# etemesi254/zune-jpeg

Measured on AMD Instinct MI355X. Metric: megapixels/sec decoded (IDCT->RGB), 4K 4:2:0 baseline, higher is better.
Workload: dtype i32

## Files before the change

### zune-jpeg_amd/csrc/zj_device.h

```cpp
#pragma once

#include <stdint.h>

#if defined(ZJ_EMU)
#define ZJ_DEV inline
#define ZJ_HD inline
#else
#include <hip/hip_runtime.h>
#define ZJ_DEV __device__ __forceinline__
#define ZJ_HD __host__ __device__ __forceinline__
#endif

namespace zj {

typedef uint16_t u16x2 __attribute__((vector_size(4)));
typedef int16_t s16x2 __attribute__((vector_size(4)));

#if defined(ZJ_EMU)
#define ZJ_GLOBAL_PTR(T, v) (reinterpret_cast<T*>(v))
#else
#define ZJ_GLOBAL_PTR(T, v) ((T*)(__attribute__((address_space(1))) T*)(v))
#endif

struct alignas(16) U4 { uint32_t x, y, z, w; };
struct alignas(8) U2 { uint32_t x, y; };
typedef uint32_t V4 __attribute__((vector_size(16)));
#if defined(ZJ_ABLATION)
#define ZJ_ABL(debug, bit) ((debug) & (bit))
#define ZJ_PDBG(p) ((p).debug)
#else
#define ZJ_ABL(debug, bit) 0
#define ZJ_PDBG(p) 0
#endif
#ifndef ZJ_NT
#define ZJ_NT 4
#endif
#ifndef ZJ_SEAM_WB
#define ZJ_SEAM_WB 0
#endif
#ifndef ZJ_ROUND_ROT
#define ZJ_ROUND_ROT 1
#endif

#ifndef ZJ_CBYTE
#define ZJ_CBYTE 1
#endif
#ifndef ZJ_INTERIOR
#define ZJ_INTERIOR 1
#endif

ZJ_DEV uint32_t as_u32(u16x2 v) { uint32_t r; __builtin_memcpy(&r, &v, 4); return r; }
ZJ_DEV uint32_t as_u32(s16x2 v) { uint32_t r; __builtin_memcpy(&r, &v, 4); return r; }
ZJ_DEV u16x2 as_u16x2(uint32_t v) { u16x2 r; __builtin_memcpy(&r, &v, 4); return r; }
ZJ_DEV s16x2 as_s16x2(uint32_t v) { s16x2 r; __builtin_memcpy(&r, &v, 4); return r; }

#if !defined(ZJ_EMU)
extern "C" __device__ __attribute__((const)) int zj_llvm_mul_i24(int, int) __asm("llvm.amdgcn.mul.i24");
#endif
ZJ_DEV int32_t mul24(int32_t a, int32_t b)
{
#if defined(ZJ_EMU)
    int32_t a24 = (int32_t)((uint32_t)a << 8) >> 8, b24 = (int32_t)((uint32_t)b << 8) >> 8;
    return (int32_t)((uint32_t)a24 * (uint32_t)b24);
#else
    return zj_llvm_mul_i24(a, b);
#endif
}
ZJ_DEV int32_t wadd(int32_t a, int32_t b) { return (int32_t)((uint32_t)a + (uint32_t)b); }
ZJ_DEV int32_t wsub(int32_t a, int32_t b) { return (int32_t)((uint32_t)a - (uint32_t)b); }
ZJ_DEV int32_t mad24(int32_t a, int32_t b, int32_t c) { return wadd(mul24(a, b), c); }
ZJ_DEV int32_t wshl(int32_t a, int s) { return (int32_t)((uint32_t)a << s); }

ZJ_DEV int32_t dot2(uint32_t a, uint32_t k, int32_t c)
{
#if defined(ZJ_EMU)
    const int32_t al = (int16_t)(a & 0xffff), ah = (int16_t)(a >> 16), bl = (int16_t)(k & 0xffff), bh = (int16_t)(k >> 16);
    return (int32_t)((uint32_t)(al * bl) + (uint32_t)(ah * bh) + (uint32_t)c);
#else
    int32_t r;
    asm("v_dot2_i32_i16 %0, %1, %2, %3" : "=v"(r) : "v"(a), "s"(k), "v"(c));
    return r;
#endif
}
ZJ_DEV int32_t dot2z(uint32_t a, uint32_t k)
{
#if defined(ZJ_EMU)
    return dot2(a, k, 0);
#else
    int32_t r;
    asm("v_dot2_i32_i16 %0, %1, %2, 0" : "=v"(r) : "v"(a), "s"(k));
    return r;
#endif
}
constexpr uint32_t pk16(int lo, int hi) { return ((uint32_t)lo & 0xffffu) | (((uint32_t)hi & 0xffffu) << 16); }

ZJ_DEV uint32_t sad_u16(uint32_t a, uint32_t b, uint32_t c)
{
#if defined(ZJ_EMU)
    const int32_t al = (int32_t)(a & 0xffff), ah = (int32_t)(a >> 16), bl = (int32_t)(b & 0xffff), bh = (int32_t)(b >> 16);
    return (uint32_t)((al > bl ? al - bl : bl - al) + (ah > bh ? ah - bh : bh - ah)) + c;
#else
// ... 240 lines not shown
#pragma unroll
        for (int g = 0; g < G; g++)
#pragma unroll
            for (int k = 0; k < 8; k += 2) {
                const uint32_t hi = perm((uint32_t)o[g][k + 1], (uint32_t)o[g][k], 0x07060302u);
                const s16x2 z = {0, 0}, m = {255, 255};
                ow[(r0 + g) * 4 + (k >> 1)] = as_u32(pk_min(pk_max(sar(as_u16x2(hi), 1), z), m));
            }
        ZJ_SCHED_BARRIER();
    }
}

struct PackedHalf { int32_t x0, x1, x2, x3, u0, u1, u2, u3; };
ZJ_DEV PackedHalf idct_1d_dot(const uint32_t p04, const uint32_t p26, const uint32_t p13, const uint32_t p57, const int32_t bias)
{
    PackedHalf h;
    const int32_t t0 = dot2(p04, pk16(4096, 4096), bias);
    const int32_t t1 = dot2(p04, pk16(4096, -4096), bias);
    h.x0 = dot2(p26, pk16(5352, 2217), t0);
    h.x3 = dot2(p26, pk16(-5352, -2217), t0);
    h.x1 = dot2(p26, pk16(2217, -5350), t1);
    h.x2 = dot2(p26, pk16(-2217, 5350), t1);
    h.u3 = dot2(p57, pk16(3219, 1131), dot2z(p13, pk16(5683, 4816)));
    h.u2 = dot2(p57, pk16(-5681, -3218), dot2z(p13, pk16(4816, -1129)));
    h.u1 = dot2(p57, pk16(1132, 4816), dot2z(p13, pk16(3219, -5681)));
    h.u0 = dot2(p57, pk16(4816, -5680), dot2z(p13, pk16(1131, -3218)));
    return h;
}
ZJ_DEV void idct_1d_dot_add(const PackedHalf& h, int32_t o[8])
{
    o[0] = wadd(h.x0, h.u3); o[7] = wsub(h.x0, h.u3);
    o[1] = wadd(h.x1, h.u2); o[6] = wsub(h.x1, h.u2);
    o[2] = wadd(h.x2, h.u1); o[5] = wsub(h.x2, h.u1);
    o[3] = wadd(h.x3, h.u0); o[4] = wsub(h.x3, h.u0);
}

ZJ_DEV int classify_block(const uint32_t* w, const uint32_t* g)
{
    uint32_t any = w[0] & 0xffff0000u;
#pragma unroll
    for (int i = 1; i < 32; i++) any |= w[i];
    if (any == 0) return 0;
    int32_t bad = 0;
#pragma unroll
    for (int jj = 0; jj < 4; jj++) {
        uint32_t st = 0, sb = 0;
#pragma unroll
        for (int k = 0; k < 4; k++) st = sad_u16(w[4 * k + jj], 0x80008000u, st);
#pragma unroll
        for (int k = 4; k < 8; k++) sb = sad_u16(w[4 * k + jj], 0x80008000u, sb);
        const int32_t d = mad24((int32_t)g[4 + jj], (int32_t)sb, mad24((int32_t)g[jj], (int32_t)st, -(int32_t)g[8 + jj]));
        bad |= d;
    }
    return bad < 0 ? 2 : 1;
}

ZJ_DEV void idct_block_packed(const U4 raw[8], const uint32_t* qp, uint32_t out[16])
{
    const uint32_t* w = reinterpret_cast<const uint32_t*>(raw);
    uint32_t D[32];
#pragma unroll
    for (int i = 0; i < 32; i++) D[i] = as_u32(as_u16x2(w[i]) * as_u16x2(qp[i]));
    uint32_t T[8][4];
#pragma unroll
    for (int g = 0; g < 4; g++) {
        const int ca = g == 0 ? 0 : (g == 1 ? 2 : (g == 2 ? 1 : 5)), cb = g == 0 ? 4 : (g == 1 ? 6 : (g == 2 ? 3 : 7));
        PackedHalf h[2];
#pragma unroll
        for (int e = 0; e < 2; e++) {
            const int col = e ? cb : ca, jj = col >> 1;
            const uint32_t sel = (col & 1) ? 0x07060302u : 0x05040100u;
            const uint32_t p04 = perm(D[4 * 4 + jj], D[0 * 4 + jj], sel), p26 = perm(D[6 * 4 + jj], D[2 * 4 + jj], sel);
            const uint32_t p13 = perm(D[3 * 4 + jj], D[1 * 4 + jj], sel), p57 = perm(D[7 * 4 + jj], D[5 * 4 + jj], sel);
            h[e] = idct_1d_dot(p04, p26, p13, p57, 512);
        }
        ZJ_SCHED_BARRIER();
        int32_t oa[8], ob[8];
        idct_1d_dot_add(h[0], oa);
        idct_1d_dot_add(h[1], ob);
#pragma unroll
        for (int i = 0; i < 8; i++) T[i][g] = pack_sar<10>(oa[i], ob[i]);
        ZJ_SCHED_BARRIER();
    }
    constexpr int32_t bias2 = 512 + 65536 + (128 << 17);
#pragma unroll
    for (int r0 = 0; r0 < 8; r0 += 2) {
        PackedHalf h[2];
#pragma unroll
        for (int e = 0; e < 2; e++) h[e] = idct_1d_dot(T[r0 + e][0], T[r0 + e][1], T[r0 + e][2], T[r0 + e][3], bias2);
        ZJ_SCHED_BARRIER();
#pragma unroll
        for (int e = 0; e < 2; e++) {
            int32_t o[8];
            idct_1d_dot_add(h[e], o);
            out[2 * (r0 + e)] = sat_pk_u8_2(pack_sar<17>(o[0], o[1]), pack_sar<17>(o[2], o[3]));
            out[2 * (r0 + e) + 1] = sat_pk_u8_2(pack_sar<17>(o[4], o[5]), pack_sar<17>(o[6], o[7]));
        }
        ZJ_SCHED_BARRIER();
    }
}

ZJ_DEV uint32_t dc_only_value(uint32_t w0, int32_t q0, const int clamp = 0)
{
    const int16_t dc = (int16_t)(uint16_t)((uint32_t)lo16s(w0) * (uint32_t)(int32_t)(int16_t)q0);
    int32_t v = ((int32_t)dc >> 3) + 128;
    if (clamp) v = v < 0 ? 0 : (v > 255 ? 255 : v);
// ... 56 lines not shown
#define ZJ_TWC_GRAY 128
#endif
#ifndef ZJ_NT_MIN_GRAY
#define ZJ_NT_MIN_GRAY 256
#endif
template <> struct TileWidth<1, 1, false> { static constexpr int TWC = ZJ_TWC_GRAY; };

enum { OUT_RGB = 0, OUT_GRAY = 1, OUT_YCBCR = 2, OUT_RGBA = 3, OUT_RGB_CHW = 4 };
enum { GEN_WIDE = 0, GEN_PACKED = 1 };

template <int HS, int VS, int OUT>
struct Cfg {
    static constexpr bool CHROMA = OUT != OUT_GRAY;
    static constexpr int YBR = (HS == 2 && VS == 2) ? 4 : ((HS == 2 || VS == 2) ? 2 : 1);
    static constexpr int CBR = (HS == 2) ? 2 : 1;
    static constexpr int SH = YBR * 8;
    static constexpr int CROWS = CBR * 8;
    static constexpr int TWC = TileWidth<HS, VS, CHROMA>::TWC;
    static constexpr int HALO = (HS == 2) ? 1 : 0;
    static constexpr int TWYB = TWC * HS;
    static constexpr int TWY = TWYB * 8;
    static constexpr int NYB = YBR * TWYB;
    static constexpr int CCOLS = TWC + 2 * HALO;
    static constexpr int NCB = CBR * CCOLS;
    static constexpr int CPITCH = TWC * 8;
    static constexpr int COFF = 0;
    static constexpr int YSZ = SH * TWY;
    static constexpr int CSZ = CROWS * CPITCH;
    static constexpr int NGRP = TWY / 16;
    static constexpr int NITEMS = SH * NGRP;
    static constexpr int NBLK = NYB + (CHROMA ? 2 * NCB : 0);
    static constexpr int NT_BLK = (NBLK + 63) / 64 * 64;
    static constexpr int NT_MIN = (HS == 1 && VS == 1) ? (CHROMA ? ZJ_NT_MIN_444 : ZJ_NT_MIN_GRAY) : ((HS == 2 && VS == 1 && CHROMA) ? ZJ_NT_MIN_H : ((HS == 2 && VS == 2 && CHROMA) ? ZJ_NT_MIN_HV : ((HS == 1 && VS == 2 && CHROMA) ? ZJ_NT_MIN_V : 0)));
    static constexpr int NT = NT_BLK > NT_MIN ? NT_BLK : NT_MIN;
    static constexpr int NW = NT / 64;
    static constexpr int ROUND_ROT = (ZJ_ROUND_ROT && NITEMS % NT != 0 && NITEMS % NT <= 64 && NW > 1) ? 1 : 0;

    static constexpr int LUT_N = SH + 2;
    static constexpr int LUT_BYTES = ((2 * LUT_N * 2 + 15) / 16) * 16;
    static constexpr int HRAW = (CHROMA && HALO) ? 2 * 2 * CROWS : 0;
    static constexpr int HFIL = (CHROMA && HALO) ? 2 * 2 * SH : 0;
    static constexpr bool TSCAP = OUT == OUT_RGB || OUT == OUT_YCBCR || OUT == OUT_RGBA;
    static constexpr int PPI = OUT == OUT_RGBA ? 4 : 3;
    static constexpr int INPL = 64 / PPI * PPI;
    static constexpr int XSTAGE = ((64 * PPI - INPL) * 16 + 31) / 32 * 32;
    static constexpr bool HALO_PURE = CHROMA && HALO && (NYB + 2 * CBR * TWC) % 64 == 0 && 2 * CBR * 2 * 8 == 64;
    static constexpr int HALO_T0 = NYB + 2 * CBR * TWC;
#if defined(ZJ_EMU) && !defined(ZJ_EMU_REDO_ANY)
    static constexpr bool CBYTE_OUT = OUT == OUT_RGB || OUT == OUT_RGBA || OUT == OUT_RGB_CHW;
#else
    static constexpr bool CBYTE_OUT = true;
#endif
    static constexpr bool CBYTE = ZJ_CBYTE != 0 && CHROMA && HS == 2 && HALO_PURE && NGRP == 16 && NYB % 64 == 0 && CBYTE_OUT;
    static constexpr bool INTERIOR = ZJ_INTERIOR != 0 && CBYTE && TSCAP && NITEMS % NT == 0 && ROUND_ROT == 0;
    template <int GEN> struct L {
        static constexpr int YPX = GEN == GEN_PACKED ? 1 : 2;
        static constexpr bool CB = GEN == GEN_PACKED && CBYTE;
        static constexpr int CPX = CB ? 1 : 2;
        static constexpr int CPB = CPITCH * CPX;
        static constexpr int CPLANE = CROWS * CPB;
        static constexpr int CBYTES = CHROMA ? 2 * CPLANE + (HRAW + HFIL) * 2 : 0;
        static_assert(CBYTES % 16 == 0, "tables stay 16-byte aligned");
        static constexpr int C_OFF = GEN == GEN_PACKED ? (NITEMS + 63) / 64 * 64 * 16 : YSZ * 2;
        static constexpr int HRAW_OFF = C_OFF + 2 * CPLANE;
        static constexpr int HFIL_OFF = HRAW_OFF + HRAW * 2;
        static constexpr int TAB_OFF = C_OFF + CBYTES;
        static constexpr int LUT_OFF = TAB_OFF + TAB_BYTES;
        static constexpr int FLAG_OFF = LUT_OFF + LUT_BYTES;
        static constexpr int X_OFF = FLAG_OFF + 16;
        static constexpr int X_STAGE = TSCAP ? NW * XSTAGE : 0;
        static constexpr int X_HALO = HALO_PURE ? 8 * 80 * 4 : 0;
        static constexpr int BYTES = GEN == GEN_PACKED ? X_OFF + (X_STAGE > X_HALO ? X_STAGE : X_HALO) : FLAG_OFF;
        static_assert(C_OFF % 16 == 0 && TAB_OFF % 16 == 0, "16-byte alignment of the planes");
    };
    static constexpr int LDS_WIDE = L<GEN_WIDE>::BYTES;
    static constexpr int LDS_PACKED = L<GEN_PACKED>::BYTES > LDS_WIDE ? L<GEN_PACKED>::BYTES : LDS_WIDE;
    static constexpr int PIECES_PER_ROW = PPI * NGRP;
    static constexpr int PPR_MAGIC = (1 << 20) / PIECES_PER_ROW + 1;
    static constexpr bool ppr_magic_ok()
    {
        for (int q = 0; q < PPI * ((NITEMS + NT - 1) / NT * NT) + 64 * PPI; q++)
            if ((int)(((unsigned)q * (unsigned)PPR_MAGIC) >> 20) != q / PIECES_PER_ROW) return false;
        return true;
    }
    static_assert(ppr_magic_ok(), "PPR_MAGIC");
    static_assert(NT <= 512 && NBLK <= NT, "one lane per block, at most 8 waves");
};

constexpr int SCATTER_MAX = 32;

struct Params {
    const int16_t* y;
    const int16_t* cb;
    const int16_t* cr;
    uint8_t* out;
    long long y_frame_stride;
    long long c_frame_stride;
    long long out_frame_stride;
    int width, height;
    int mcu_x;
    int n_strips;
    int tiles_per_row;
    int regular_px;
    int nframes;
    int zero_fill;
    int total_tiles;
    uint32_t tpr_magic, tpr_shift;
// ... 296 lines not shown
template <class C>
ZJ_DEV void halo_pass2(const HaloLane& H, char* lds, const int clamp_dc)
{
    const int32_t* sc = lds_halo_scratch<C>(lds, H.hb);
    const int i = H.j;
    const U4 f0 = *reinterpret_cast<const U4*>(sc + 64), f1 = *reinterpret_cast<const U4*>(sc + 68);
    const uint32_t any = f0.x | f0.y | f0.z | f0.w | f1.x | f1.y | f1.z | f1.w;
    int32_t v;
    if (any == 0) {
        const uint16_t* q = reinterpret_cast<const uint16_t*>(lds_tab<C, GEN_PACKED>(lds) + TAB_DW * H.comp);
        v = (int32_t)(int16_t)(dc_only_value((uint32_t)sc[72], (int32_t)q[0], clamp_dc) & 0xffffu);
        if (C::template L<GEN_PACKED>::CB && (uint32_t)v > 255u) *lds_flag<C>(lds) = 1;
    } else {
        const U4 a = *reinterpret_cast<const U4*>(sc + 8 * i), b = *reinterpret_cast<const U4*>(sc + 8 * i + 4);
        const int32_t t0 = (int32_t)a.x, t1 = (int32_t)a.y, t2 = (int32_t)a.z, t3 = (int32_t)a.w;
        const int32_t t4 = (int32_t)b.x, t5 = (int32_t)b.y, t6 = (int32_t)b.z, t7 = (int32_t)b.w;
        constexpr int32_t bias2 = 512 + 65536 + (128 << 17);
        int32_t x0 = mad24(t2, 2217 + 3135, wadd(wshl(wadd(t0, t4), 12), bias2));
        x0 = mad24(t6, 2217, x0);
        int32_t u3 = mul24(t1, 6149 + 4816 - 3685 - 1597);
        u3 = mad24(t7, 4816 - 3685, u3);
        u3 = mad24(t5, 4816 - 1597, u3);
        u3 = mad24(t3, 4816, u3);
        v = (H.last_col ? wsub(x0, u3) : wadd(x0, u3)) >> 17;
        v = v < 0 ? 0 : (v > 255 ? 255 : v);
    }
    *reinterpret_cast<int16_t*>(H.dst + i * H.pitch) = (int16_t)v;
}

template <class C, int HS, int VS, int GEN>
ZJ_DEV int halo_value(char* lds, const int comp, const int side, const int m, const bool wrap)
{
    const int16_t* raw = lds_halo_raw<C, GEN>(lds, comp, side, 0);
    if (VS == 2) {
        const int16_t* lut = lds_lut<C, GEN>(lds);
        const int i = m + 1 + (wrap ? (side == 0 ? -1 : 1) : 0);
        const int ra = lut[i] / C::template L<GEN>::CPB, rb = lut[C::LUT_N + i] / C::template L<GEN>::CPB;
        return tri1(raw[ra], raw[rb]);
    }
    const int r = side == 0 ? (wrap && m > 0 ? m - 1 : m) : (wrap && m < C::SH - 1 ? m + 1 : m);
    return raw[r];
}
template <class C, int HS, int VS>
ZJ_DEV void halo_filter(const Params& p, const TileId t, const int hl, char* lds)
{
    const int cbw = p.mcu_x, cb0 = t.tile * C::TWC;
    const bool left_wrap = cb0 == 0, right_wrap = cb0 + C::TWC >= cbw;
    for (int q = hl; q < C::HFIL; q += 64) {
        const int comp = 1 + q / (2 * C::SH), side = (q / C::SH) & 1, m = q % C::SH;
        *lds_halo_fil<C, GEN_PACKED>(lds, comp, side, m) = (int16_t)halo_value<C, HS, VS, GEN_PACKED>(lds, comp, side, m, side == 0 ? left_wrap : right_wrap);
    }
}

template <class C, int GEN, bool NEED_Y16>
ZJ_DEV void finish_block(const BlockLoc& L, const U4 raw[8], char* lds, const int debug = 0, const int clamp_dc = 0)
{
    if (!L.valid) return;
    const uint32_t* w = reinterpret_cast<const uint32_t*>(raw);
    const uint32_t* tab = lds_tab<C, GEN>(lds) + TAB_DW * L.comp;
    if (GEN == GEN_WIDE) {
        uint32_t any = w[0] & 0xffff0000u;
#pragma unroll
        for (int i = 1; i < 32; i++) any |= w[i];
        if (any != 0 && !ZJ_ABL(debug, 1)) {
            U4 px[8];
            idct_block(raw, reinterpret_cast<const uint16_t*>(tab), px);
            store_block(L, px);
        } else {
            store_splat(L, dc_only_value(w[0], (int32_t)(tab[0] & 0xffffu), clamp_dc));
        }
        return;
    }
    using LLp = typename C::template L<GEN_PACKED>;
    constexpr bool CB = LLp::CB;
    constexpr bool CONST_PITCH = C::HALO_PURE && (CB || C::TWY * LLp::YPX == LLp::CPB);
    BlockLoc Lc = L;
    if (CONST_PITCH) { Lc.pitch = LLp::CPB; Lc.halo = 0; }
    const int ypitch = CONST_PITCH ? C::TWY * LLp::YPX : L.pitch;
    int cls = classify_block(w, tab + 32);
    if (ZJ_ABL(debug, 1)) cls = 0;
    if (cls == 0) {
        const uint32_t v = dc_only_value(w[0], (int32_t)(tab[0] & 0xffffu), clamp_dc);
        if (L.comp != 0 && !CB) { store_splat(Lc, v); return; }
        if ((L.comp != 0 || NEED_Y16) && (v & 0xffffu) > 255u) *lds_flag<C>(lds) = 1;
        const uint32_t b = (v & 0xffu) * 0x01010101u;
        const U2 row = {b, b};
        if (L.comp != 0) {
#pragma unroll
            for (int r = 0; r < 8; r++) *reinterpret_cast<U2*>(Lc.dst + r * Lc.pitch) = row;
            return;
        }
#pragma unroll
        for (int r = 0; r < 8; r++) *reinterpret_cast<U2*>(Lc.dst + r * ypitch) = row;
        return;
    }
    auto emit = [&](const uint32_t* b) {
        if (L.comp == 0) {
#pragma unroll
            for (int r = 0; r < 8; r++) { const U2 row = {b[2 * r], b[2 * r + 1]}; *reinterpret_cast<U2*>(Lc.dst + r * ypitch) = row; }
        } else if (CB) {
#pragma unroll
            for (int r = 0; r < 8; r++) { const U2 row = {b[2 * r], b[2 * r + 1]}; *reinterpret_cast<U2*>(Lc.dst + r * Lc.pitch) = row; }
        } else {
            U4 px[8];
            bytes_to_rows(b, px);
            store_block(Lc, px);
        }
    };
    if (cls == 1) {
        uint32_t b[16];
        idct_block_packed(raw, tab, b);
        emit(b);
        return;
    }
    {
        ZJ_NO_IF_CONVERT();
        uint32_t b[16];
        U4 px[8];
        idct_block(raw, reinterpret_cast<const uint16_t*>(tab), px);
        rows_to_bytes(px, b);
        emit(b);
    }
}

ZJ_DEV void store16(uint8_t* p, const U4& v, const bool staged = false)
{
#if !defined(ZJ_EMU)
    if ((ZJ_NT & 1) || ((ZJ_NT & 4) && staged)) { const V4 t = {v.x, v.y, v.z, v.w}; __builtin_nontemporal_store(t, reinterpret_cast<V4*>(p)); return; }
#endif
#if defined(ZJ_EMU)
    __builtin_memcpy(p, &v, 16);
#else
// ... 113 lines not shown
    return (q < C::INPL ? ybase : xbase) + 16 * q;
}

template <class C, int VS>
ZJ_DEV void nb_pair(const uint32_t vm[4], const char* cp, const int oa, const int ob, const int lc, const int g, uint32_t& prev, uint32_t& next,
                    const uint32_t pl = 0, const uint32_t nr = 0)
{
#if !defined(ZJ_EMU)
    if (C::NGRP == 16) {
        prev = (uint32_t)__builtin_amdgcn_update_dpp((int)pl, (int)vm[3], 0x111, 0xf, 0xf, false);
        next = (uint32_t)__builtin_amdgcn_update_dpp((int)nr, (int)vm[0], 0x101, 0xf, 0xf, false);
        return;
    }
#endif
    prev = next = 0;
    if (g > 0) {
        prev = *reinterpret_cast<const uint32_t*>(cp + oa + lc - 4);
        if (VS == 2) prev = tri(prev, *reinterpret_cast<const uint32_t*>(cp + ob + lc - 4));
    }
    if (g < C::NGRP - 1) {
        next = *reinterpret_cast<const uint32_t*>(cp + oa + lc + 16);
        if (VS == 2) next = tri(next, *reinterpret_cast<const uint32_t*>(cp + ob + lc + 16));
    }
}

template <class C, int VS>
ZJ_DEV void nb_bytes(const uint32_t a0, const uint32_t a1, const char* cp, const int oa, const int ob, const int lc, const int g,
                     uint32_t& prev, uint32_t& next, const uint32_t pl, const uint32_t nr)
{
#if !defined(ZJ_EMU)
    if (C::NGRP == 16) {
        prev = (uint32_t)__builtin_amdgcn_update_dpp((int)pl, (int)a1, 0x111, 0xf, 0xf, false);
        next = (uint32_t)__builtin_amdgcn_update_dpp((int)nr, (int)a0, 0x101, 0xf, 0xf, false);
        return;
    }
#endif
    prev = next = 0;
    if (g > 0) {
        prev = *reinterpret_cast<const uint32_t*>(cp + oa + lc - 4);
        if (VS == 2) prev = tri_b(prev, *reinterpret_cast<const uint32_t*>(cp + ob + lc - 4));
    }
    if (g < C::NGRP - 1) {
        next = *reinterpret_cast<const uint32_t*>(cp + oa + lc + 8);
        if (VS == 2) next = tri_b(next, *reinterpret_cast<const uint32_t*>(cp + ob + lc + 8));
    }
}

template <class C>
ZJ_DEV bool interior_tile(const Params& p, const TileId t)
{
    const int cb0 = t.tile * C::TWC;
    return cb0 != 0 && cb0 + C::TWC < p.mcu_x && p.height - t.strip * C::SH >= C::SH && p.edge_rep == 0;
}

template <class C, bool INTERIOR = false>
ZJ_DEV void stage_item(const ItemOut& io, const int tid , char* lds, const int round, const int hw_wave = -1)
{
    if (!INTERIOR && io.kind == 0) return;
    const int lwave = tid >> 6, lane = tid & 63;
    const int item0 = 64 * lwave + round * C::NT;
    const int wave = hw_wave < 0 ? lwave : hw_wave;
    if (!INTERIOR && C::PPI == 3 && io.kind == 3) {
        const U4 z = {0, 0, 0, 0};
        *reinterpret_cast<U4*>(piece_addr<C>(lds, item0, wave, 3 * lane - 1)) = io.s0;
        *reinterpret_cast<U4*>(piece_addr<C>(lds, item0, wave, 3 * lane)) = io.s1;
        *reinterpret_cast<U4*>(piece_addr<C>(lds, item0, wave, 3 * lane + 1)) = io.s2;
        *reinterpret_cast<U4*>(piece_addr<C>(lds, item0, wave, 3 * lane + 2)) = z;
        return;
    }
    U4* const dst = reinterpret_cast<U4*>(piece_addr<C>(lds, item0, wave, C::PPI * lane));
    dst[0] = io.s0;
    dst[1] = io.s1;
    if (C::PPI == 4) { dst[2] = io.s2; dst[3] = io.s3; }
    else if (INTERIOR || io.kind == 1) dst[2] = io.s2;
}

template <class C, int HS, int VS, int OUT, int GEN, bool FAST = true, bool TS = false, bool RAG = false, bool INTERIOR = false>
ZJ_DEV void phase_color(const Params& p, const TileId t, const int tid, char* lds, const int round = 0, ItemOut* io = nullptr)
{
    using LL = typename C::template L<GEN>;
    static_assert(!INTERIOR || (TS && FAST && !RAG && GEN == GEN_PACKED && LL::CB && C::INTERIOR), "the interior form exists for the staged byte-chroma rounds");
    const int P = p.mcu_x * 8 * HS;
    const int W = p.width;
    const int cbw = p.mcu_x;
    const int cb0 = t.tile * C::TWC;
    const int nvalid = INTERIOR ? C::TWC : ((cbw - cb0) < C::TWC ? (cbw - cb0) : C::TWC);
    const bool left_wrap = !INTERIOR && cb0 == 0, right_wrap = !INTERIOR && cb0 + C::TWC >= cbw;
    const bool edge_tile = HS == 2 && (left_wrap || right_wrap);
    const int x0 = t.tile * C::TWY;
    const long long row_bytes = p.out_pitch;
    uint8_t* const frame_out = t.out;
    const int elements = P / 16 - 1;
    if (TS) io->kind = 0;

    for (int item = TS ? tid + round * C::NT : tid; item < C::NITEMS; item += TS ? C::NITEMS : C::NT) {
        const int m = item / C::NGRP, g = item % C::NGRP;
        const int px0 = x0 + 16 * g;
        const int row = t.strip * C::SH + m;
        if (!INTERIOR && (px0 >= P || row >= p.height)) continue;
        const bool irregular = RAG && px0 >= p.regular_px;
        uint8_t* const orow = frame_out + (long long)row * row_bytes;
        uint32_t yp[8];
        if (GEN == GEN_PACKED) {
            const U4 yv = *reinterpret_cast<const U4*>(lds + 16 * item);
            if (OUT == OUT_GRAY) {
                if (FAST && !irregular) store16(orow + px0, yv, true);
                else { const uint32_t ow4[4] = {yv.x, yv.y, yv.z, yv.w}; store_clip(orow, px0, ow4, 4, W, 0, 0); }
                continue;
            }
            const uint32_t yb[4] = {yv.x, yv.y, yv.z, yv.w};
#pragma unroll
            for (int k = 0; k < 4; k++) {
                if (HS == 2) { yp[k] = perm(0, yb[k], 0x0c020c00u); yp[4 + k] = perm(0, yb[k], 0x0c030c01u); }
                else { yp[2 * k] = perm(0, yb[k], 0x0c010c00u); yp[2 * k + 1] = perm(0, yb[k], 0x0c030c02u); }
            }
        } else {
            const U4* yrow = reinterpret_cast<const U4*>(lds + 32 * item);
            const U4 ya = yrow[0], yb = yrow[1];
            const uint32_t yw[8] = {ya.x, ya.y, ya.z, ya.w, yb.x, yb.y, yb.z, yb.w};
            if (OUT == OUT_GRAY) {
                U4 o;
                o.x = perm(yw[1], yw[0], 0x06040200u); o.y = perm(yw[3], yw[2], 0x06040200u);
                o.z = perm(yw[5], yw[4], 0x06040200u); o.w = perm(yw[7], yw[6], 0x06040200u);
                if (FAST && !irregular) store16(orow + px0, o);
                else { const uint32_t ow4[4] = {o.x, o.y, o.z, o.w}; store_clip(orow, px0, ow4, 4, W, 0, 0); }
                continue;
            }
            if (HS == 2) {
#pragma unroll
                for (int k = 0; k < 4; k++) {
                    yp[k] = perm(yw[2 * k + 1], yw[2 * k], 0x05040100u);
                    yp[4 + k] = perm(yw[2 * k + 1], yw[2 * k], 0x07060302u);
                }
            } else {
#pragma unroll
                for (int k = 0; k < 8; k++) yp[k] = yw[k];
            }
        }

        uint32_t cbp[8], crp[8];
        bool first = false, last = false;
        int oa, ob;
        if (VS == 2) {
            const int16_t* lut = lds_lut<C, GEN>(lds);
            oa = lut[m + 1]; ob = lut[C::LUT_N + m + 1];
        } else {
            oa = ob = m * LL::CPB;
        }
        if (edge_tile) {
            ZJ_NO_IF_CONVERT();
            first = (g == 0) && left_wrap;
            last = (8 * g + 8 == 8 * nvalid) && right_wrap;
        }
        const bool rep_first = first && p.edge_rep, rep_last = last && p.edge_rep;
        const bool no_left = first && m == 0 && !p.edge_rep, no_right = last && m == C::SH - 1 && !p.edge_rep;
#pragma unroll
        for (int ch = 0; ch < 2; ch++) {
            const char* cp = lds + LL::C_OFF + ch * LL::CPLANE;
            uint32_t* dst = ch ? crp : cbp;
            if (ZJ_ABL(ZJ_PDBG(p), 16)) {
#pragma unroll
                for (int k = 0; k < 8; k++) dst[k] = yp[k] + ch;
                continue;
            }
            if (HS == 1) {
                const U4* A = reinterpret_cast<const U4*>(cp + oa + 32 * g);
                const U4 a0 = A[0], a1 = A[1];
                uint32_t v[8] = {a0.x, a0.y, a0.z, a0.w, a1.x, a1.y, a1.z, a1.w};
                if (VS == 2) {
                    const U4* B = reinterpret_cast<const U4*>(cp + ob + 32 * g);
                    const U4 b0 = B[0], b1 = B[1];
                    const uint32_t f[8] = {b0.x, b0.y, b0.z, b0.w, b1.x, b1.y, b1.z, b1.w};
#pragma unroll
                    for (int k = 0; k < 8; k++) v[k] = tri(v[k], f[k]);
                }
#pragma unroll
                for (int k = 0; k < 8; k++) dst[k] = v[k];
            } else if (LL::CB) {
                const int lc = C::COFF + 8 * g;
                const U2 a = *reinterpret_cast<const U2*>(cp + oa + lc);
                uint32_t a0 = a.x, a1 = a.y;
                if (VS == 2) {
                    const U2 b = *reinterpret_cast<const U2*>(cp + ob + lc);
                    a0 = tri_b(a0, b.x); a1 = tri_b(a1, b.y);
                }
                uint32_t prev, next;
                {
                    const int hvl = *lds_halo_fil<C, GEN>(lds, ch + 1, 0, m), hvr = *lds_halo_fil<C, GEN>(lds, ch + 1, 1, m);
                    const uint32_t pl = (uint32_t)hvl << 24, nr = (uint32_t)hvr & 0xffu;
                    nb_bytes<C, VS>(a0, a1, cp, oa, ob, lc, g, prev, next, pl, nr);
#if defined(ZJ_EMU)
                    constexpr bool DPP_ENDS = false;
#else
                    constexpr bool DPP_ENDS = C::NGRP == 16;
#endif
                    if (!DPP_ENDS) {
                        if (g == 0) prev = pl;
                        if (g == nvalid - 1) next = nr;
                    } else if (!INTERIOR && nvalid != C::NGRP) {
                        ZJ_NO_IF_CONVERT();
                        if (g == nvalid - 1) next = nr;
                    }
                }
                if (!INTERIOR && p.edge_rep) {
                    ZJ_NO_IF_CONVERT();
                    if (rep_first) prev = a0 << 24;
                    if (rep_last) next = a1 >> 24;
                }
                const uint32_t l0 = alignbyte(a0, prev, 3), l1 = alignbyte(a1, a0, 3);
                const uint32_t r0 = alignbyte(a1, a0, 1), r1 = alignbyte(next, a1, 1);
                uint32_t e0 = tri_b(a0, l0), e1 = tri_b(a1, l1);
                uint32_t o0 = tri_b(a0, r0), o1 = tri_b(a1, r1);
                if (edge_tile) {
                    ZJ_NO_IF_CONVERT();
                    if (no_left) e0 = (e0 & 0xffffff00u) | (a0 & 0xffu);
                    if (no_right) {
                        e1 = (e1 & 0x00ffffffu) | ((o1 << 8) & 0xff000000u);
                        o1 = (o1 & 0x00ffffffu) | (a1 & 0xff000000u);
                    }
                }
                dst[0] = perm(0, e0, 0x0c010c00u); dst[1] = perm(0, e0, 0x0c030c02u);
                dst[2] = perm(0, e1, 0x0c010c00u); dst[3] = perm(0, e1, 0x0c030c02u);
                dst[4] = perm(0, o0, 0x0c010c00u); dst[5] = perm(0, o0, 0x0c030c02u);
                dst[6] = perm(0, o1, 0x0c010c00u); dst[7] = perm(0, o1, 0x0c030c02u);
            } else {
                const int lc = (C::COFF + 8 * g) * 2;
                const U4 a = *reinterpret_cast<const U4*>(cp + oa + lc);
                uint32_t vm[4] = {a.x, a.y, a.z, a.w};
                if (VS == 2) {
                    const U4 b = *reinterpret_cast<const U4*>(cp + ob + lc);
                    vm[0] = tri(vm[0], b.x); vm[1] = tri(vm[1], b.y);
                    vm[2] = tri(vm[2], b.z); vm[3] = tri(vm[3], b.w);
                }
                uint32_t prev, next;
                {
                    int hvl, hvr;
                    if (GEN == GEN_PACKED && C::HALO_PURE) {
                        hvl = *lds_halo_fil<C, GEN>(lds, ch + 1, 0, m);
                        hvr = *lds_halo_fil<C, GEN>(lds, ch + 1, 1, m);
                    } else {
                        hvl = halo_value<C, HS, VS, GEN>(lds, ch + 1, 0, m, left_wrap);
                        hvr = halo_value<C, HS, VS, GEN>(lds, ch + 1, 1, m, right_wrap);
                    }
                    const uint32_t pl = (uint32_t)hvl << 16, nr = (uint32_t)hvr & 0xffffu;
                    nb_pair<C, VS>(vm, cp, oa, ob, lc, g, prev, next, pl, nr);
#if defined(ZJ_EMU)
                    constexpr bool DPP_ENDS = false;
#else
                    constexpr bool DPP_ENDS = C::NGRP == 16;
#endif
                    if (!DPP_ENDS) {
                        if (g == 0) prev = pl;
                        if (g == nvalid - 1) next = nr;
                    } else if (nvalid != C::NGRP) {
                        ZJ_NO_IF_CONVERT();
                        if (g == nvalid - 1) next = nr;
                    }
                }
                if (p.edge_rep) {
                    ZJ_NO_IF_CONVERT();
                    if (rep_first) prev = vm[0] << 16;
                    if (rep_last) next = vm[3] >> 16;
                }
#pragma unroll
                for (int k = 0; k < 4; k++) {
                    const uint32_t L = align16(vm[k], k == 0 ? prev : vm[k - 1]);
// ... 61 lines not shown
#pragma unroll
        for (int k = 0; k < 4; k++) {
            if (HS == 2) pack_rgb4_eo(c[k], c[4 + k], d[3 * k], d[3 * k + 1], d[3 * k + 2]);
            else pack_rgb4_nat(c[2 * k], c[2 * k + 1], d[3 * k], d[3 * k + 1], d[3 * k + 2]);
        }
        if (!FAST || (irregular && !TS)) {
#pragma unroll
            for (int h = 0; h < 2; h++) store_unit_generic<OUT>(p, orow, P, (px0 >> 3) + h, d + 6 * h);
            continue;
        }
        const U4 s0 = {d[0], d[1], d[2], d[3]}, s1 = {d[4], d[5], d[6], d[7]}, s2 = {d[8], d[9], d[10], d[11]};
        if (ZJ_ABL(ZJ_PDBG(p), 8) && (d[0] ^ d[5] ^ d[11]) != 0x12345u) continue;
        const int G = px0 >> 4;
        const bool quirk = OUT == OUT_RGB && !p.plain && !RAG;
        if (TS) {
            io->s0 = s0; io->s1 = s1; io->s2 = s2;
            io->kind = INTERIOR ? 1 : ((quirk && G == elements) ? 3 : ((quirk && G == elements - 1) ? 2 : 1));
            continue;
        }
        if (!quirk) {
            uint8_t* o = orow + 48ll * G;
            store16(o, s0); store16(o + 16, s1); store16(o + 32, s2);
        } else {
            if (G < elements - 1) {
                uint8_t* o = orow + 48ll * G;
                store16(o, s0); store16(o + 16, s1); store16(o + 32, s2);
            } else if (G == elements - 1) {
                uint8_t* o = orow + 48ll * G;
                store16(o, s0); store16(o + 16, s1);
            } else {
                uint8_t* o = orow + 3ll * W - 64;
                store16(o, s0); store16(o + 16, s1); store16(o + 32, s2);
                if (p.zero_fill) { const U4 z = {0, 0, 0, 0}; store16(o + 48, z); }
            }
        }
    }
}

template <class C, int OUT, bool RAG = false, bool SEAM = false, bool INTERIOR = false>
ZJ_DEV void color_copyout(const Params& p, const TileId t, const int tid , char* lds, const int round, const int hw_wave = -1)
{
    using LL = typename C::template L<GEN_PACKED>;
    static_assert(!INTERIOR || (!RAG && !SEAM && C::INTERIOR), "the interior form exists for the plain staged rounds");
    constexpr int PPI = C::PPI;
    const int P = RAG ? p.regular_px : p.mcu_x * 8 * (C::TWYB / C::TWC);
    const int x0 = t.tile * C::TWY;
    const int left = P - x0 > 0 ? (P - x0) / 16 : 0;
    const int nvg = left < C::NGRP ? left : C::NGRP;
    const uint32_t row_bytes = (uint32_t)p.out_pitch;
    uint8_t* const tile_out = t.out + (long long)t.strip * C::SH * row_bytes + (long long)(PPI == 4 ? 4 : 3) * x0;
    const int w = uniform(tid >> 6), L = tid & 63;
    const int item0 = 64 * w + round * C::NT;
    if (!INTERIOR && item0 >= C::NITEMS) return;
    const bool row_end_here = !RAG && x0 + 16 * nvg == P;
    const int never = (OUT == OUT_RGB && !p.plain && !p.zero_fill && row_end_here) ? 3 * nvg - 1 : -1;
    const int rows_left = p.height - t.strip * C::SH;
    const char* const ybase = lds + 16 * item0;
    const char* const xbase = lds + LL::X_OFF + C::XSTAGE * (hw_wave < 0 ? w : hw_wave) - 16 * C::INPL;
    const char* src[PPI];
    uint32_t off[PPI];
    int mm[PPI], cc[PPI];
    constexpr bool WHOLE_ROWS = C::NT % C::NGRP == 0;
    const int item_q = WHOLE_ROWS ? 64 * w : item0;
    const int row_shift = WHOLE_ROWS ? round * (C::NT / C::NGRP) : 0;
#pragma unroll
    for (int j = 0; j < PPI; j++) {
        src[j] = (j == 0 && L < C::INPL ? ybase : xbase) + 16 * (64 * j + L);
        const int Q = PPI * item_q + 64 * j + L;
        const int m0 = (int)(((uint32_t)Q * (uint32_t)C::PPR_MAGIC) >> 20);
        cc[j] = Q - m0 * C::PIECES_PER_ROW;
        mm[j] = m0 + row_shift;
        off[j] = (uint32_t)mul24(m0, (int32_t)row_bytes) + 16u * (uint32_t)cc[j] + (uint32_t)row_shift * row_bytes;
    }
    const bool plain_round = INTERIOR || (nvg == C::NGRP && rows_left >= C::SH && never < 0 && item0 + 64 <= C::NITEMS);
    static_assert(!(SEAM && RAG), "the seam form serves aligned widths");
    uint32_t la0 = 0, lrho = 0, segb = 0;
    if (SEAM) { la0 = (uint32_t)reinterpret_cast<uintptr_t>(tile_out) & 127u; lrho = row_bytes & 127u; segb = 16u * (uint32_t)(PPI * nvg); }
    const bool seams = SEAM && (la0 | lrho) != 0;
    auto shared_line = [&](const int j) {
        const uint32_t A = (la0 + (uint32_t)mm[j] * lrho) & 127u, ls = (A + 16u * (uint32_t)cc[j]) & ~127u;
        return ls < A || ls + 128u > A + segb;
    };
    if (RAG) {
        const uint32_t a0 = (uint32_t)reinterpret_cast<uintptr_t>(tile_out) & 3u, rho = row_bytes & 3u;
        if ((a0 | rho) != 0) {
            ZJ_NO_IF_CONVERT();
#pragma unroll
            for (int j = 0; j < PPI; j++) {
                const bool ok = plain_round || (PPI * item0 + 64 * j + L < PPI * C::NITEMS && cc[j] < PPI * nvg && mm[j] < rows_left);
                const bool last = cc[j] == PPI * nvg - 1;
                const uint32_t delta = (4u - ((a0 + (uint32_t)mm[j] * rho) & 3u)) & 3u;
                const U4 v = *reinterpret_cast<const U4*>(src[j]);
                const int qn = 64 * j + L + 1;
                const char* const src2 = last ? src[j] : (qn < C::INPL ? ybase : xbase) + 16 * qn;
                const uint32_t nx = *reinterpret_cast<const uint32_t*>(src2);
                U4 o;
                o.x = alignbyte(v.y, v.x, delta); o.y = alignbyte(v.z, v.y, delta);
                o.z = alignbyte(v.w, v.z, delta); o.w = alignbyte(nx, v.w, delta);
                uint8_t* const dst = tile_out + off[j];
                if (ok) {
                    if (!last) store16(dst + delta, o, true);
                    else {
                        uint32_t* const d32 = reinterpret_cast<uint32_t*>(dst + delta);
                        d32[0] = o.x; d32[1] = o.y; d32[2] = o.z;
                        if (delta == 0) d32[3] = o.w;
                        else for (uint32_t b = 0; b < 4u - delta; b++) dst[delta + 12 + b] = (uint8_t)(o.w >> (8 * b));
// ... 214 lines not shown
```

### zune-jpeg_amd/csrc/zj_kernels.hip

```cpp
#include <hip/hip_runtime.h>
#include <atomic>
#include <stdio.h>

#include "zj_device.h"
#include "zj_launch.h"

#ifndef ZJ_WAVES_PER_SIMD
#define ZJ_WAVES_PER_SIMD 5
#endif
#ifndef ZJ_WAVES_PER_SIMD_PACKED
#define ZJ_WAVES_PER_SIMD_PACKED 6
#endif

namespace zj {

#ifndef ZJ_PRIO
#define ZJ_PRIO 1
#endif
#define ZJ_SETPRIO(bit, level) do { if (ZJ_PRIO & (bit)) __builtin_amdgcn_s_setprio(level); } while (0)

template <class C, int HS, int VS, int OUT, bool FAST, bool RAG = false>
__device__ __forceinline__ void tile_wide(const Params& p, const TileId t, const int tid, char* lds)
{
    ZJ_SETPRIO(1, 3);
    const BlockLoc L = locate<C, GEN_WIDE>(p, t, tid, lds);
    U4 raw[8];
    load_block(L, raw, ZJ_PDBG(p));
    ZJ_SETPRIO(1, 0);
    phase_setup<C, HS, VS, GEN_WIDE>(p, tid, lds);
    __syncthreads();
    finish_block<C, GEN_WIDE, false>(L, raw, lds, ZJ_PDBG(p), p.clamp_dc);
    __syncthreads();
    ZJ_SETPRIO(2, 2);
    phase_color<C, HS, VS, OUT, GEN_WIDE, FAST, false, RAG>(p, t, tid, lds);
}

template <class C, int HS, int VS, int OUT>
__device__ __forceinline__ void interior_rounds(const Params& p, const TileId t, const int tid, char* lds)
{
    static_assert(C::ROUND_ROT == 0, "full rounds: the logical thread numbering is the hardware's");
    __builtin_assume(tid >= 0 && tid < C::NT);
#pragma unroll
    for (int round = 0; round * C::NT < C::NITEMS; round++) {
        ItemOut io;
        phase_color<C, HS, VS, OUT, GEN_PACKED, true, true, false, true>(p, t, tid, lds, round, &io);
        if (round == 0 && ZJ_ABL(ZJ_PDBG(p), 128)) { ZJ_USE(io.s0.x ^ io.s0.y ^ io.s0.z ^ io.s0.w ^ io.s1.x ^ io.s1.y ^ io.s1.z ^ io.s1.w ^ io.s2.x ^ io.s2.y ^ io.s2.z ^ io.s2.w); return; }
        stage_item<C, true>(io, tid, lds, round);
        ZJ_WAVE_FENCE();
        color_copyout<C, OUT, false, false, true>(p, t, tid, lds, round);
        ZJ_WAVE_FENCE();
        if (round == 0 && ZJ_ABL(ZJ_PDBG(p), 256)) return;
    }
}

__device__ __forceinline__ void stagger_start(const Params& p, const int bid)
{
    if (p.stagger_delay <= 0 || bid >= p.stagger_wgs) return;
    const Magic g = {p.stagger_magic, p.stagger_shift};
    const int k = (int)magic_div((uint32_t)bid, g);
    const int n = k * p.stagger_delay;
    for (int i = 0; i < n; i++) __builtin_amdgcn_s_sleep(2);
}

#ifndef ZJ_ASSUME_NO_HALO
#define ZJ_ASSUME_NO_HALO 1
#endif
#ifndef ZJ_PIN_ARGS
#define ZJ_PIN_ARGS 1
#endif
__device__ __forceinline__ void pin_head(const Params& p)
{
    if (!ZJ_PIN_ARGS) return;
    asm volatile("; kernel arguments 0x00-0x87 are resident"
                 :: "s"(p.y), "s"(p.cb), "s"(p.cr), "s"(p.out), "s"(p.y_frame_stride), "s"(p.c_frame_stride), "s"(p.out_frame_stride),
                    "s"(p.width), "s"(p.height), "s"(p.mcu_x), "s"(p.n_strips), "s"(p.tiles_per_row), "s"(p.regular_px), "s"(p.zero_fill),
                    "s"(p.total_tiles), "s"(p.tpr_magic), "s"(p.tpr_shift), "s"(p.ns_magic), "s"(p.ns_shift), "s"(p.stagger_wgs),
                    "s"(p.stagger_delay), "s"(p.stagger_magic), "s"(p.stagger_shift), "s"(p.plain), "s"(p.out_pitch));
}

template <int HS, int VS, int OUT, int GEN, bool FAST, bool TS, bool RAG, bool SEAM = false>
__device__ __forceinline__ void fused_body(const Params& p, char* lds)
{
    using C = Cfg<HS, VS, OUT>;
    pin_head(p);
    const TileId t = decode_tile(p, (int)blockIdx.x);
#ifndef ZJ_ROTATE
#define ZJ_ROTATE 0
#endif
#ifndef ZJ_ROLE_SHIFT
#define ZJ_ROLE_SHIFT 0
#endif
    int tid = (int)threadIdx.x;
    if ((ZJ_ROTATE || ZJ_ROLE_SHIFT) && C::NW > 1) {
        const unsigned b = blockIdx.x;
        const int rot = ZJ_ROTATE ? (int)((b ^ (b >> 3) ^ (b >> 8)) % (unsigned)C::NW) : ZJ_ROLE_SHIFT % C::NW;
        tid += 64 * rot;
        if ((C::NT & (C::NT - 1)) == 0) tid &= C::NT - 1; else if (tid >= C::NT) tid -= C::NT;
        __builtin_assume(tid >= 0 && tid < C::NT);
    }
    stagger_start(p, (int)blockIdx.x);
    if (GEN == GEN_WIDE) { tile_wide<C, HS, VS, OUT, FAST, RAG>(p, t, tid, lds); return; }
    constexpr bool NEED_Y16 = OUT == OUT_RGB || OUT == OUT_RGBA || OUT == OUT_RGB_CHW;
    ZJ_SETPRIO(1, 3);
    const bool halo_wave = C::HALO_PURE && (__builtin_amdgcn_readfirstlane(tid) >> 6) == C::HALO_T0 / 64;
    if (halo_wave) {
        HaloLane H = halo_locate<C>(p, t, tid - C::HALO_T0, lds);
        int32_t hs8[8];
        halo_load(H, hs8);
        ZJ_SETPRIO(1, 0);
        phase_setup<C, HS, VS, GEN_PACKED>(p, tid, lds);
        if (ZJ_ABL(ZJ_PDBG(p), 32)) return;
        __syncthreads();
        halo_pass1<C>(H, hs8, lds);
        ZJ_WAVE_FENCE();
        halo_pass2<C>(H, lds, p.clamp_dc);
        ZJ_WAVE_FENCE();
        halo_filter<C, HS, VS>(p, t, tid - C::HALO_T0, lds);
    } else {
        if (ZJ_ASSUME_NO_HALO && C::HALO_PURE && C::NT == C::HALO_T0 + 64) __builtin_assume(tid < C::HALO_T0);
        const BlockLoc L = locate<C, GEN_PACKED>(p, t, tid, lds);
        U4 raw[8];
        load_block(L, raw, ZJ_PDBG(p));
        ZJ_SETPRIO(1, 0);
        phase_setup<C, HS, VS, GEN_PACKED>(p, tid, lds);
        if (ZJ_ABL(ZJ_PDBG(p), 32)) return;
        __syncthreads();
        finish_block<C, GEN_PACKED, NEED_Y16>(L, raw, lds, ZJ_PDBG(p), p.clamp_dc);
    }
    __builtin_amdgcn_s_waitcnt(0x0f70);
    if (ZJ_ABL(ZJ_PDBG(p), 64)) return;
    __syncthreads();
    const bool redo = (NEED_Y16 || C::CBYTE) && __builtin_amdgcn_readfirstlane((int)*lds_flag<C>(lds)) != 0;
    if (redo) {
        __syncthreads();
        tile_wide<C, HS, VS, OUT, FAST, RAG>(p, t, tid, lds);
    } else if (TS) {
        ZJ_SETPRIO(2, 2);
        __builtin_amdgcn_s_waitcnt(0x0f70);
        constexpr bool INTERIOR = C::INTERIOR && FAST && !RAG && !SEAM;
        if constexpr (INTERIOR) {
            if (interior_tile<C>(p, t)) { interior_rounds<C, HS, VS, OUT>(p, t, tid, lds); return; }
        }
#pragma unroll
        for (int round = 0; round * C::NT < C::NITEMS; round++) {
            ItemOut io;
            const int hw = C::ROUND_ROT ? uniform(tid >> 6) : -1, ltid = round_tid<C>(tid, round);
            phase_color<C, HS, VS, OUT, GEN_PACKED, FAST, true, RAG>(p, t, ltid, lds, round, &io);
            if (round == 0 && ZJ_ABL(ZJ_PDBG(p), 128)) { ZJ_USE(io.s0.x ^ io.s0.y ^ io.s0.z ^ io.s0.w ^ io.s1.x ^ io.s1.y ^ io.s1.z ^ io.s1.w ^ io.s2.x ^ io.s2.y ^ io.s2.z ^ io.s2.w); return; }
            stage_item<C>(io, ltid, lds, round, hw);
            ZJ_WAVE_FENCE();
            color_copyout<C, OUT, RAG, SEAM>(p, t, ltid, lds, round, hw);
            ZJ_WAVE_FENCE();
            if (round == 0 && ZJ_ABL(ZJ_PDBG(p), 256)) return;
        }
    } else {
        ZJ_SETPRIO(2, 2);
        __builtin_amdgcn_s_waitcnt(0x0f70);
        phase_color<C, HS, VS, OUT, GEN_PACKED, FAST, false, RAG>(p, t, tid, lds);
    }
}

template <int HS, int VS, int OUT, int GEN, bool FAST, bool TS>
__global__ __launch_bounds__((Cfg<HS, VS, OUT>::NT), (GEN == GEN_PACKED ? ZJ_WAVES_PER_SIMD_PACKED : ZJ_WAVES_PER_SIMD)) void zj_fused_kernel(const Params p)
{
    using C = Cfg<HS, VS, OUT>;
    __shared__ __attribute__((aligned(16))) char lds[GEN == GEN_PACKED ? C::LDS_PACKED : C::LDS_WIDE];
    fused_body<HS, VS, OUT, GEN, FAST, TS, false>(p, lds);
}

template <int HS, int VS, int OUT>
__global__ __launch_bounds__((Cfg<HS, VS, OUT>::NT), ZJ_WAVES_PER_SIMD_PACKED) void zj_fused_seam_kernel(const Params p)
{
    using C = Cfg<HS, VS, OUT>;
    __shared__ __attribute__((aligned(16))) char lds[C::LDS_PACKED];
    fused_body<HS, VS, OUT, GEN_PACKED, true, C::TSCAP, false, C::TSCAP>(p, lds);
}

#ifndef ZJ_WAVES_PER_SIMD_RAG
#define ZJ_WAVES_PER_SIMD_RAG ZJ_WAVES_PER_SIMD_PACKED
#endif
template <int HS, int VS, int OUT, bool TS>
__global__ __launch_bounds__((Cfg<HS, VS, OUT>::NT), ZJ_WAVES_PER_SIMD_RAG) void zj_fused_ragged_kernel(const Params p)
{
    using C = Cfg<HS, VS, OUT>;
    __shared__ __attribute__((aligned(16))) char lds[C::LDS_PACKED];
    fused_body<HS, VS, OUT, GEN_PACKED, true, TS, true>(p, lds);
}

__global__ __launch_bounds__(256) void zj_zero_rows_kernel(const ZeroRows z)
{
    const int fr = (int)blockIdx.y / z.nr, r = (int)blockIdx.y - fr * z.nr;
    uint8_t* const base = (z.out ? z.out + (long long)fr * z.frame_stride : ZJ_GLOBAL_PTR(uint8_t, z.fptr[fr])) + z.off[r];
    const unsigned long long len = z.len[r], begin = (unsigned long long)blockIdx.x * 16384ull;
    if (begin >= len) return;
// ... 268 lines not shown
```

Before: 965,700.

## Add SAD-based block classifier, row-wise interior copyout, and first-tile interior path

Three changes. A new block classifier reuses the SAD sums it already computes to detect DC-only blocks, replacing the separate OR-reduction over all coefficients. The interior copyout now writes whole rows per wave with a fixed per-lane address formula instead of the general edge-aware path. Tiles in the first column now take the interior round path with a simplified left-edge fix, so fewer tiles fall back to the generic edge handling. Together these aim to cut ALU and branch work in the fast path, at the cost of more template specialisations and code size.

```diff
diff --git a/zune-jpeg_amd/csrc/zj_device.h b/zune-jpeg_amd/csrc/zj_device.h
--- a/zune-jpeg_amd/csrc/zj_device.h
+++ b/zune-jpeg_amd/csrc/zj_device.h
@@ -47,6 +47,16 @@
 #endif
 #ifndef ZJ_INTERIOR
 #define ZJ_INTERIOR 1
+#endif
+
+#ifndef ZJ_CLS_SAD
+#define ZJ_CLS_SAD 1
+#endif
+#ifndef ZJ_COPY_ROWS
+#define ZJ_COPY_ROWS 1
+#endif
+#ifndef ZJ_FIRST
+#define ZJ_FIRST 1
 #endif
 
 ZJ_DEV uint32_t as_u32(u16x2 v) { uint32_t r; __builtin_memcpy(&r, &v, 4); return r; }
@@ -393,6 +403,24 @@
         const int32_t d = mad24((int32_t)g[4 + jj], (int32_t)sb, mad24((int32_t)g[jj], (int32_t)st, -(int32_t)g[8 + jj]));
         bad |= d;
     }
+    return bad < 0 ? 2 : 1;
+}
+ZJ_DEV int classify_block_sad(const uint32_t* w, const uint32_t* g)
+{
+    int32_t bad = 0;
+    uint32_t all = 0;
+#pragma unroll
+    for (int jj = 0; jj < 4; jj++) {
+        uint32_t st = 0, sb = 0;
+#pragma unroll
+        for (int k = 0; k < 4; k++) st = sad_u16(w[4 * k + jj], 0x80008000u, st);
+#pragma unroll
+        for (int k = 4; k < 8; k++) sb = sad_u16(w[4 * k + jj], 0x80008000u, sb);
+        all += st + sb;
+        bad |= mad24((int32_t)g[4 + jj], (int32_t)sb, mad24((int32_t)g[jj], (int32_t)st, -(int32_t)g[8 + jj]));
+    }
+    const uint32_t dc = sad_u16(w[0] & 0xffffu, 0x00008000u, 0u);
+    if (all - dc == 8u * 262144u - 32768u) return 0;
     return bad < 0 ? 2 : 1;
 }
 
@@ -555,7 +583,8 @@
     static constexpr bool CBYTE_OUT = true;
 #endif
     static constexpr bool CBYTE = ZJ_CBYTE != 0 && CHROMA && HS == 2 && HALO_PURE && NGRP == 16 && NYB % 64 == 0 && CBYTE_OUT;
-    static constexpr bool INTERIOR = ZJ_INTERIOR != 0 && CBYTE && TSCAP && NITEMS % NT == 0 && ROUND_ROT == 0;
+    static constexpr bool FRONT = CBYTE && TSCAP && NITEMS % NT == 0 && ROUND_ROT == 0;
+    static constexpr bool INTERIOR = ZJ_INTERIOR != 0 && FRONT;
     template <int GEN> struct L {
         static constexpr int YPX = GEN == GEN_PACKED ? 1 : 2;
         static constexpr bool CB = GEN == GEN_PACKED && CBYTE;
@@ -958,7 +987,7 @@
     }
 }
 
-template <class C, int GEN, bool NEED_Y16>
+template <class C, int GEN, bool NEED_Y16, bool FRONT = false>
 ZJ_DEV void finish_block(const BlockLoc& L, const U4 raw[8], char* lds, const int debug = 0, const int clamp_dc = 0)
 {
     if (!L.valid) return;
@@ -983,7 +1012,7 @@
     BlockLoc Lc = L;
     if (CONST_PITCH) { Lc.pitch = LLp::CPB; Lc.halo = 0; }
     const int ypitch = CONST_PITCH ? C::TWY * LLp::YPX : L.pitch;
-    int cls = classify_block(w, tab + 32);
+    int cls = (FRONT && ZJ_CLS_SAD) ? classify_block_sad(w, tab + 32) : classify_block(w, tab + 32);
     if (ZJ_ABL(debug, 1)) cls = 0;
     if (cls == 0) {
         const uint32_t v = dc_only_value(w[0], (int32_t)(tab[0] & 0xffffu), clamp_dc);
@@ -1203,6 +1232,11 @@
     const int cb0 = t.tile * C::TWC;
     return cb0 != 0 && cb0 + C::TWC < p.mcu_x && p.height - t.strip * C::SH >= C::SH && p.edge_rep == 0;
 }
+template <class C>
+ZJ_DEV bool first_tile(const Params& p, const TileId t)
+{
+    return t.tile == 0 && C::TWC < p.mcu_x && p.height - t.strip * C::SH >= C::SH && p.edge_rep == 0;
+}
 
 template <class C, bool INTERIOR = false>
 ZJ_DEV void stage_item(const ItemOut& io, const int tid , char* lds, const int round, const int hw_wave = -1)
@@ -1226,11 +1260,12 @@
     else if (INTERIOR || io.kind == 1) dst[2] = io.s2;
 }
 
-template <class C, int HS, int VS, int OUT, int GEN, bool FAST = true, bool TS = false, bool RAG = false, bool INTERIOR = false>
+template <class C, int HS, int VS, int OUT, int GEN, bool FAST = true, bool TS = false, bool RAG = false, bool INTERIOR = false, bool FIRST = false>
 ZJ_DEV void phase_color(const Params& p, const TileId t, const int tid, char* lds, const int round = 0, ItemOut* io = nullptr)
 {
     using LL = typename C::template L<GEN>;
     static_assert(!INTERIOR || (TS && FAST && !RAG && GEN == GEN_PACKED && LL::CB && C::INTERIOR), "the interior form exists for the staged byte-chroma rounds");
+    static_assert(!FIRST || INTERIOR, "the first-tile form is an interior form");
     const int P = p.mcu_x * 8 * HS;
     const int W = p.width;
     const int cbw = p.mcu_x;
@@ -1304,7 +1339,7 @@
             last = (8 * g + 8 == 8 * nvalid) && right_wrap;
         }
         const bool rep_first = first && p.edge_rep, rep_last = last && p.edge_rep;
-        const bool no_left = first && m == 0 && !p.edge_rep, no_right = last && m == C::SH - 1 && !p.edge_rep;
+        const bool no_left = FIRST ? item == 0 : (first && m == 0 && !p.edge_rep), no_right = last && m == C::SH - 1 && !p.edge_rep;
 #pragma unroll
         for (int ch = 0; ch < 2; ch++) {
             const char* cp = lds + LL::C_OFF + ch * LL::CPLANE;
@@ -1362,7 +1397,9 @@
                 const uint32_t r0 = alignbyte(a1, a0, 1), r1 = alignbyte(next, a1, 1);
                 uint32_t e0 = tri_b(a0, l0), e1 = tri_b(a1, l1);
                 uint32_t o0 = tri_b(a0, r0), o1 = tri_b(a1, r1);
-                if (edge_tile) {
+                if (FIRST) {
+                    if (no_left) e0 = (e0 & 0xffffff00u) | (a0 & 0xffu);
+                } else if (edge_tile) {
                     ZJ_NO_IF_CONVERT();
                     if (no_left) e0 = (e0 & 0xffffff00u) | (a0 & 0xffu);
                     if (no_right) {
@@ -1530,6 +1567,24 @@
     const int w = uniform(tid >> 6), L = tid & 63;
     const int item0 = 64 * w + round * C::NT;
     if (!INTERIOR && item0 >= C::NITEMS) return;
+    if constexpr (INTERIOR && ZJ_COPY_ROWS != 0) {
+        constexpr int PPR = C::PIECES_PER_ROW, RPW = 64 / C::NGRP;
+        static_assert(64 % C::NGRP == 0 && RPW * PPR == 64 * PPI && PPR >= 32, "a wave's round is whole rows; one boundary per 64 pieces at most");
+        const uint32_t step = row_bytes - 16u * (uint32_t)PPR;
+        uint8_t* const wave_out = tile_out + (unsigned long long)(uint32_t)(item0 / C::NGRP) * row_bytes;
+        const uint32_t l16 = 16u * (uint32_t)L;
+        U4 v[PPI];
+#pragma unroll
+        for (int j = 0; j < PPI; j++) v[j] = *reinterpret_cast<const U4*>((j == 0 && L < C::INPL ? lds + 16 * item0 : lds + LL::X_OFF + C::XSTAGE * w - 16 * C::INPL) + 16 * (64 * j + L));
+#pragma unroll
+        for (int j = 0; j < PPI; j++) {
+            const int RJ = 64 * j / PPR, TJ = (RJ + 1) * PPR - 64 * j;
+            uint8_t* const base = wave_out + (1024u * (uint32_t)j + (uint32_t)RJ * step);
+            const uint32_t voff = TJ < 64 ? l16 + (L >= TJ ? step : 0u) : l16;
+            store16(base + voff, v[j], true);
+        }
+        return;
+    }
     const bool row_end_here = !RAG && x0 + 16 * nvg == P;
     const int never = (OUT == OUT_RGB && !p.plain && !p.zero_fill && row_end_here) ? 3 * nvg - 1 : -1;
     const int rows_left = p.height - t.strip * C::SH;
diff --git a/zune-jpeg_amd/csrc/zj_kernels.hip b/zune-jpeg_amd/csrc/zj_kernels.hip
--- a/zune-jpeg_amd/csrc/zj_kernels.hip
+++ b/zune-jpeg_amd/csrc/zj_kernels.hip
@@ -35,7 +35,7 @@
     phase_color<C, HS, VS, OUT, GEN_WIDE, FAST, false, RAG>(p, t, tid, lds);
 }
 
-template <class C, int HS, int VS, int OUT>
+template <class C, int HS, int VS, int OUT, bool FIRST = false>
 __device__ __forceinline__ void interior_rounds(const Params& p, const TileId t, const int tid, char* lds)
 {
     static_assert(C::ROUND_ROT == 0, "full rounds: the logical thread numbering is the hardware's");
@@ -43,7 +43,7 @@
 #pragma unroll
     for (int round = 0; round * C::NT < C::NITEMS; round++) {
         ItemOut io;
-        phase_color<C, HS, VS, OUT, GEN_PACKED, true, true, false, true>(p, t, tid, lds, round, &io);
+        phase_color<C, HS, VS, OUT, GEN_PACKED, true, true, false, true, FIRST>(p, t, tid, lds, round, &io);
         if (round == 0 && ZJ_ABL(ZJ_PDBG(p), 128)) { ZJ_USE(io.s0.x ^ io.s0.y ^ io.s0.z ^ io.s0.w ^ io.s1.x ^ io.s1.y ^ io.s1.z ^ io.s1.w ^ io.s2.x ^ io.s2.y ^ io.s2.z ^ io.s2.w); return; }
         stage_item<C, true>(io, tid, lds, round);
         ZJ_WAVE_FENCE();
@@ -82,6 +82,7 @@
 __device__ __forceinline__ void fused_body(const Params& p, char* lds)
 {
     using C = Cfg<HS, VS, OUT>;
+    constexpr bool FRONT = C::FRONT && GEN == GEN_PACKED && FAST && TS && !RAG && !SEAM;
     pin_head(p);
     const TileId t = decode_tile(p, (int)blockIdx.x);
 #ifndef ZJ_ROTATE
@@ -125,7 +126,7 @@
         phase_setup<C, HS, VS, GEN_PACKED>(p, tid, lds);
         if (ZJ_ABL(ZJ_PDBG(p), 32)) return;
         __syncthreads();
-        finish_block<C, GEN_PACKED, NEED_Y16>(L, raw, lds, ZJ_PDBG(p), p.clamp_dc);
+        finish_block<C, GEN_PACKED, NEED_Y16, FRONT>(L, raw, lds, ZJ_PDBG(p), p.clamp_dc);
     }
     __builtin_amdgcn_s_waitcnt(0x0f70);
     if (ZJ_ABL(ZJ_PDBG(p), 64)) return;
@@ -140,6 +141,9 @@
         constexpr bool INTERIOR = C::INTERIOR && FAST && !RAG && !SEAM;
         if constexpr (INTERIOR) {
             if (interior_tile<C>(p, t)) { interior_rounds<C, HS, VS, OUT>(p, t, tid, lds); return; }
+            if constexpr (ZJ_FIRST != 0) {
+                if (first_tile<C>(p, t)) { interior_rounds<C, HS, VS, OUT, true>(p, t, tid, lds); return; }
+            }
         }
 #pragma unroll
         for (int round = 0; round * C::NT < C::NITEMS; round++) {
```

Result: no change. 965,100 (-0.1%).
